# taithenguyen/ppls

Hardware: AMD Instinct MI355X
Metric: accepted subintervals/sec + FP64 F-evals/sec at 1/2/4/8 MI355X, EPSILON=1e-10 (higher is better)
Workload: dtype f64

## Files before the change

### ppls_amd/build.py

```python
import os
import shutil
import subprocess
import sys

HERE = os.path.dirname(os.path.abspath(__file__))
ROOT = os.path.dirname(HERE)
CSRC = os.path.join(HERE, "csrc")
OUT = os.path.join(HERE, "_build")
LIB = os.path.join(OUT, "libaquad.so")
CLI = os.path.join(OUT, "aquad")
HIPCC = shutil.which("hipcc") or "/opt/rocm/bin/hipcc"
ARCH = os.environ.get("PPLS_AMD_ARCH", "gfx950")

HIP_FLAGS = [f"--offload-arch={ARCH}", "-O3", "-std=c++17", "-ffp-contract=off", "-fPIC", "-shared",
             "-mllvm", "-amdgpu-atomic-optimizer-strategy=None",
             "-Wall", "-Wno-unused-function", "-I", os.path.join(ROOT, "include"), "-I", CSRC]

SOURCES = [os.path.join(CSRC, "aquad.hip")]
USER_F = os.path.abspath(os.environ.get("PPLS_AMD_USER_F") or os.path.join(CSRC, "plugins", "aq_user_gauss.h"))
PARAM_F = os.path.abspath(os.environ.get("PPLS_AMD_PARAM_F") or os.path.join(CSRC, "plugins", "aq_param_gauss.h"))
PLUGIN_DEFS = [f'-DAQ_USER_F_HEADER="{USER_F}"', f'-DAQ_PARAM_F_HEADER="{PARAM_F}"']
DEPS = sorted(os.path.join(CSRC, f) for f in os.listdir(CSRC) if f.endswith((".h", ".inc", ".hip"))) + \
    [os.path.join(ROOT, "include", "aquad.h"), USER_F, PARAM_F]
LIBS = ["-pthread", "-L/opt/rocm/lib", "-lrccl", "-Wl,-rpath,/opt/rocm/lib"]


def _stale(target, deps):
    if not os.path.exists(target):
        return True
    t = os.path.getmtime(target)
    return any(os.path.getmtime(d) > t for d in deps)


def build_variant(name, defines, verbose=False):
    os.makedirs(OUT, exist_ok=True)
    out = os.path.join(OUT, f"libaquad_{name}.so")
    cmd = [HIPCC] + HIP_FLAGS + PLUGIN_DEFS + list(defines) + ["-o", out] + SOURCES + LIBS
    if verbose:
        print(" ".join(cmd))
    subprocess.check_call(cmd)
    return out


def build(force=False, verbose=False):
    os.makedirs(OUT, exist_ok=True)
    tab = os.path.join(CSRC, "aq_exp_table.h")
    if not os.path.exists(tab):
        subprocess.check_call([sys.executable, os.path.join(CSRC, "gen_exp_table.py")])
    if not os.path.exists(os.path.join(CSRC, "aq_sincos_table.h")):
        subprocess.check_call([sys.executable, os.path.join(CSRC, "gen_sincos_table.py")])
    if force or _stale(LIB, DEPS):
        cmd = [HIPCC] + HIP_FLAGS + PLUGIN_DEFS + ["-o", LIB] + SOURCES + LIBS
        if verbose:
            print(" ".join(cmd))
        subprocess.check_call(cmd)
    cli_src = os.path.join(CSRC, "aquad_cli.c")
    if os.path.exists(cli_src) and (force or _stale(CLI, [cli_src, LIB])):
        cmd = ["gcc", "-O2", "-std=gnu11", "-Wall", "-I", os.path.join(ROOT, "include"), "-o", CLI, cli_src,
               "-L", OUT, "-laquad", "-Wl,-rpath,$ORIGIN", "-lm"]
        if verbose:
            print(" ".join(cmd))
        subprocess.check_call(cmd)
    return LIB


if __name__ == "__main__":
    if "--variant" in sys.argv:
        i = sys.argv.index("--variant")
        extra = []
        for a in sys.argv[i + 2:]:
            if a.startswith("-D"):
                extra.append(a)
            elif a.startswith("--mllvm="):
                extra += ["-mllvm", a[len("--mllvm="):]]
            elif a.startswith("-f"):
                extra.append(a)
        print("built", build_variant(sys.argv[i + 1], extra))
    else:
        build(force="--force" in sys.argv, verbose=True)
        print("built", LIB)
```

### ppls_amd/csrc/aq_device.h

```cpp
#pragma once
#include <hip/hip_runtime.h>
#include <stdint.h>

#include <type_traits>

#include "aquad.h"
#include "aq_libm.h"

#pragma clang fp contract(off)

namespace aq {

enum : unsigned { ERRB_TIMEOUT = 1, ERRB_OVERFLOW = 2, ERRB_DEPTH = 4 };

__device__ __forceinline__ unsigned cu_slot() {
    const unsigned hw = __builtin_amdgcn_s_getreg((31 << 11) | 4);
    const unsigned xcc = __builtin_amdgcn_s_getreg((3 << 11) | 20);
    const unsigned cu = (hw >> 8) & 15u, sh = (hw >> 12) & 1u, se = (hw >> 13) & 7u;
    return ((xcc & 7u) << 8) | (((se << 1) | sh) << 4) | cu;
}

__device__ __forceinline__ double wave_sum(double v) {
#pragma unroll
    for (int o = 32; o > 0; o >>= 1) v += __shfl_xor(v, o, 64);
    return v;
}
__device__ __forceinline__ unsigned wave_sum_u(unsigned v) {
#pragma unroll
    for (int o = 32; o > 0; o >>= 1) v += __shfl_xor(v, o, 64);
    return v;
}
__device__ __forceinline__ unsigned wave_max_u(unsigned v) {
#pragma unroll
    for (int o = 32; o > 0; o >>= 1) v = max(v, (unsigned)__shfl_xor(v, o, 64));
    return v;
}
__device__ __forceinline__ unsigned wave_or_u(unsigned v) {
#pragma unroll
    for (int o = 32; o > 0; o >>= 1) v |= (unsigned)__shfl_xor((int)v, o, 64);
    return v;
}
__device__ __forceinline__ unsigned lane_id() { return __lane_id(); }
__device__ __forceinline__ unsigned mbcnt(unsigned long long m) {
    return __builtin_amdgcn_mbcnt_hi((unsigned)(m >> 32), __builtin_amdgcn_mbcnt_lo((unsigned)m, 0u));
}

struct Step {
    double mid, fmid, larea, rarea;
    bool refine;
};
template <int FID>
__device__ __forceinline__ Step task_step(double l, double r, double fl, double fr, double eps,
                                          const ExpEntry* __restrict__ tab, const Theta<FID>& th = Theta<FID>{}) {
    Step s;
    const double lrarea = (fl + fr) * (r - l) / 2;
    s.mid = (l + r) / 2;
    s.fmid = integrand<FID>(s.mid, tab, th);
    s.larea = (fl + s.fmid) * (s.mid - l) / 2;
    s.rarea = (s.fmid + fr) * (r - s.mid) / 2;
    s.refine = fabs((s.larea + s.rarea) - lrarea) > eps;
    return s;
}

struct Step2 {
    double fmid, area2;
    bool refine;
};
struct Step2e : Step2 {
    double diff;
};
template <typename S>
constexpr bool step_has_diff = std::is_same<S, Step2e>::value;
template <int FID>
__host__ __device__ constexpr bool doubled_areas() { return FID != F_USER && FID != F_PARAM; }
template <int FID>
__host__ __device__ constexpr double f_scale() { return FID == F_COSH4 ? 16.0 : 1.0; }
template <int FID>
__host__ __device__ constexpr double area_scale() { return doubled_areas<FID>() ? 0.5 / f_scale<FID>() : 1.0; }

template <int FID, int K, typename S = Step2>
__device__ __forceinline__ void task_step_k(const double (&l)[K], const double (&r)[K], const double (&fl)[K],
                                            const double (&fr)[K], double eps2, const ExpEntry* __restrict__ tab,
                                            S (&s)[K], const ExpConsts& kk = ExpConsts{}, int range_hint = -1,
                                            unsigned long long out_mask = 0ull, const Theta<FID>& th = Theta<FID>{}) {
    double mid[K], fmid[K];
#pragma unroll
    for (int k = 0; k < K; ++k) mid[k] = (l[k] + r[k]) / 2;
    double lr2e[K], wl[K], wr[K];
#pragma unroll
    for (int k = 0; k < K; ++k) {
        lr2e[k] = (fl[k] + fr[k]) * (r[k] - l[k]);
        wl[k] = mid[k] - l[k];
        wr[k] = r[k] - mid[k];
        asm volatile("" : "+v"(lr2e[k]), "+v"(wl[k]), "+v"(wr[k]));
    }
    integrand_k<FID, K, (f_scale<FID>() != 1.0)>(mid, fmid, tab, kk, range_hint, out_mask, th);
#pragma unroll
    for (int k = 0; k < K; ++k) {
        if constexpr (doubled_areas<FID>()) {
            const double lr2 = lr2e[k];
            const double l2 = (fl[k] + fmid[k]) * wl[k];
            const double r2 = (fmid[k] + fr[k]) * wr[k];
            s[k].fmid = fmid[k];
            s[k].area2 = l2 + r2;
            s[k].refine = fabs(s[k].area2 - lr2) > eps2;
            if constexpr (step_has_diff<S>) s[k].diff = s[k].area2 - lr2;
        } else {
            const double lrarea = (fl[k] + fr[k]) * (r[k] - l[k]) / 2;
            const double larea = (fl[k] + fmid[k]) * (mid[k] - l[k]) / 2;
            const double rarea = (fmid[k] + fr[k]) * (r[k] - mid[k]) / 2;
            s[k].fmid = fmid[k];
            s[k].area2 = larea + rarea;
            s[k].refine = fabs((larea + rarea) - lrarea) > eps2;
            if constexpr (step_has_diff<S>) s[k].diff = (larea + rarea) - lrarea;
        }
    }
}

template <int FID, unsigned TABMASK = 127u, typename S = Step2>
__device__ __forceinline__ void pair_step_halves(double ha, double hb, double fa, double fm, double fb, double eps2,
                                                 const ExpEntry* __restrict__ tab, S (&s)[2], double& m,
                                                 double& hm, const ExpConsts& kk, int range_hint,
                                                 unsigned long long out_mask, const Theta<FID>& th = Theta<FID>{}) {
    m = ha + hb;
    hm = 0.5 * m;
    const double mid[2] = {ha + hm, hm + hb};
    const double fl[2] = {fa, fm}, fr[2] = {fm, fb};
    double lr2e[2], wl[2], wr[2];
    lr2e[0] = (fa + fm) * __fma_rn(ha, -2.0, m);
    lr2e[1] = (fm + fb) * __fma_rn(hb, 2.0, -m);
    wl[0] = __fma_rn(ha, -2.0, mid[0]);
    wl[1] = mid[1] - m;
    wr[0] = m - mid[0];
    wr[1] = __fma_rn(hb, 2.0, -mid[1]);
#pragma unroll
    for (int k = 0; k < 2; ++k) asm volatile("" : "+v"(lr2e[k]), "+v"(wl[k]), "+v"(wr[k]));
    double fmid[2];
    integrand_k<FID, 2, (f_scale<FID>() != 1.0), TABMASK>(mid, fmid, tab, kk, range_hint, out_mask, th);
#pragma unroll
    for (int k = 0; k < 2; ++k) {
        s[k].fmid = fmid[k];
        if constexpr (doubled_areas<FID>()) {
            const double l2 = (fl[k] + fmid[k]) * wl[k];
            const double r2 = (fmid[k] + fr[k]) * wr[k];
            s[k].area2 = l2 + r2;
            s[k].refine = fabs(s[k].area2 - lr2e[k]) > eps2;
            if constexpr (step_has_diff<S>) s[k].diff = s[k].area2 - lr2e[k];
        } else {
            const double lrarea = lr2e[k] / 2;
            const double larea = (fl[k] + fmid[k]) * wl[k] / 2;
            const double rarea = (fmid[k] + fr[k]) * wr[k] / 2;
            s[k].area2 = larea + rarea;
            s[k].refine = fabs((larea + rarea) - lrarea) > eps2;
            if constexpr (step_has_diff<S>) s[k].diff = (larea + rarea) - lrarea;
        }
    }
}

struct Step2c {
    double fmid, l2, r2, area2;
    bool refine;
};
template <int FID>
__device__ __forceinline__ void pair_step_carry(double ha, double hb, double fa, double fm, double fb, double lr0,
                                                double lr1, double eps2, const ExpEntry* __restrict__ tab,
                                                Step2c (&s)[2], double& m, double& hm, const ExpConsts& kk,
                                                int range_hint, unsigned long long out_mask) {
    static_assert(doubled_areas<FID>(), "carried areas are doubled areas");
    m = ha + hb;
    hm = 0.5 * m;
    const double mid[2] = {ha + hm, hm + hb};
// ... 210 lines not shown
```

### ppls_amd/csrc/aq_libm.h

```cpp
#pragma once
#ifndef AQ_PIN_CONSTS
#define AQ_PIN_CONSTS 1
#endif
#include <hip/hip_runtime.h>
#include <stdint.h>

#include "aquad.h"
#include "aq_exp_table.h"
#include "aq_sincos_table.h"

#pragma clang fp contract(off)

namespace aq {

struct ExpPair {
    uint64_t tail_bits;
    uint64_t sbits;
};
static __constant__ uint64_t kExpTabBits[256] = {AQ_EXP_TAB_INIT};

struct alignas(16) ExpEntry {
    uint64_t tail_bits;
    uint64_t sbits;
};

static constexpr double kInvLn2N = 0x1.71547652b82fep7;
static constexpr double kShift = 0x1.8p52;
static constexpr double kNegLn2hiN = -0x1.62e42fefa0000p-8;
static constexpr double kNegLn2loN = -0x1.cf79abc9e3b3ap-47;
static constexpr double kC2 = 0x1.ffffffffffdbdp-2;
static constexpr double kC3 = 0x1.555555555543cp-3;
static constexpr double kC4 = 0x1.55555cf172b91p-5;
static constexpr double kC5 = 0x1.1111167a4d017p-7;

static constexpr double kQ1 = -3.33333333333331316428e-02;
static constexpr double kQ2 = 1.58730158725481460165e-03;
static constexpr double kQ3 = -7.93650757867487942473e-05;
static constexpr double kQ4 = 4.00821782732936239552e-06;
static constexpr double kQ5 = -2.01099218183624371326e-07;

__device__ __forceinline__ uint32_t hi_word(double x) {
    return (uint32_t)((uint64_t)__double_as_longlong(x) >> 32);
}

__device__ __forceinline__ double exp_glibc(double x, const ExpEntry* __restrict__ tab) {
    double kd = __fma_rn(kInvLn2N, x, kShift);
    const uint64_t ki = (uint64_t)__double_as_longlong(kd);
    kd = kd - kShift;
    const double r = __fma_rn(kd, kNegLn2loN, __fma_rn(kd, kNegLn2hiN, x));
    const ExpEntry e = tab[ki & 127];
    const double tail = __longlong_as_double((long long)e.tail_bits);
    uint64_t sbits = e.sbits + (ki << 45);
    const double r2 = r * r;
    const double tmp = __fma_rn(r2 * r2, __fma_rn(r, kC5, kC4), __fma_rn(r2, __fma_rn(r, kC3, kC2), tail + r));
    if (__builtin_expect(x >= 512.0, 0)) {
        if (x > 0x1.62e42fefa39efp+9) return __longlong_as_double(0x7ff0000000000000LL);
        sbits -= 1009ull << 52;
        const double scale = __longlong_as_double((long long)sbits);
        return 0x1p1009 * __fma_rn(scale, tmp, scale);
    }
    const double scale = __longlong_as_double((long long)sbits);
    return __fma_rn(scale, tmp, scale);
}

__device__ __forceinline__ double exp_glibc_any(double x, const ExpEntry* __restrict__ tab) {
    const uint32_t abstop = (uint32_t)((uint64_t)__double_as_longlong(x) >> 52) & 0x7ffu;
    bool special = false;
    if (__builtin_expect(abstop - 0x3c9u >= 0x408u - 0x3c9u, 0)) {
        if ((int)(abstop - 0x3c9u) < 0) return 1.0 + x;
        if (abstop >= 0x409u) {
            if (__double_as_longlong(x) == (long long)0xfff0000000000000ull) return 0.0;
            if (abstop >= 0x7ffu) return 1.0 + x;
            return x < 0.0 ? 0.0 : __longlong_as_double(0x7ff0000000000000LL);
        }
        special = true;
    }
    double kd = __fma_rn(kInvLn2N, x, kShift);
    const uint64_t ki = (uint64_t)__double_as_longlong(kd);
    kd = kd - kShift;
    const double r = __fma_rn(kd, kNegLn2loN, __fma_rn(kd, kNegLn2hiN, x));
    const ExpEntry e = tab[ki & 127];
    const double tail = __longlong_as_double((long long)e.tail_bits);
    uint64_t sbits = e.sbits + (ki << 45);
// ... 41 lines not shown
#endif
#ifndef AQ_SIN_RECIP_RN
#define AQ_SIN_RECIP_RN 1
#endif
template <int NEWTON = AQ_RCP_NEWTON>
__device__ __forceinline__ double half_recip_n(double t) {
    double y = __builtin_amdgcn_rcp(t);
    if constexpr (NEWTON == 3) {
        const double e = __fma_rn(-t, y, 1.0);
        y = __fma_rn(y, __fma_rn(e, e, e), y);
    } else {
#pragma unroll
        for (int i = 0; i < NEWTON; ++i) {
            const double e = __fma_rn(-t, y, 1.0);
            y = __fma_rn(y, e, y);
        }
    }
    const double q = 0.5 * y;
    const double r = __fma_rn(-t, q, 0.5);
    return __fma_rn(r, y, q);
}
__device__ __forceinline__ double half_recip(double t) { return half_recip_n<>(t); }
__device__ __forceinline__ double recip_rn(double x) {
    double y = __builtin_amdgcn_rcp(x);
#pragma unroll
    for (int i = 0; i < 2; ++i) {
        const double e = __fma_rn(-x, y, 1.0);
        y = __fma_rn(y, e, y);
    }
    const double r = __fma_rn(-x, y, 1.0);
    return __fma_rn(r, y, y);
}

__device__ __forceinline__ double cosh_glibc(double x, const ExpEntry* __restrict__ tab) {
    const uint32_t ix = hi_word(x) & 0x7fffffffu;
    const double ax = fabs(x);
    if (__builtin_expect(ix < 0x40360000u, 1)) {
        if (ix < 0x3fd62e43u) {
            if (ix < 0x3c800000u) return 1.0;
            const double t = expm1_glibc_small(ax);
            const double w = 1.0 + t;
            return 1.0 + (t * t) / (w + w);
        }
        const double t = exp_glibc(ax, tab);
        return __fma_rn(t, 0.5, half_recip(t));
    }
    if (ix >= 0x7ff00000u) return x * x;
    if (ix < 0x40862e42u) return 0.5 * exp_glibc(ax, tab);
    if (ax <= 0x1.633ce8fb9f87dp+9) {
        const double w = exp_glibc(0.5 * ax, tab);
        const double t = 0.5 * w;
        return t * w;
    }
    return __longlong_as_double(0x7ff0000000000000LL);
}

static __constant__ double kSinCosTab[AQ_SINCOS_TAB_N] = {AQ_SINCOS_TAB_INIT};

namespace sinc {
constexpr double s1 = -0x1.5555555555555p-3, s2 = 0.0083333333333323288, s3 = -1.9841269834414642e-04,
                 s4 = 2.755729806860771e-06, s5 = -2.5022014848318398e-08;
constexpr double sn3 = -1.66666666666664880952546298448555E-01, sn5 = 8.33333214285722277379541354343671E-03,
                 cs2 = 4.99999999999999999999950396842453E-01, cs4 = -4.16666666666664434524222570944589E-02,
                 cs6 = 1.38888874007937613028114285595617E-03;
constexpr double big = 0x1.8p45, hp0 = 0x1.921FB54442D18p0, hp1 = 0x1.1A62633145C07p-54, mp1 = 0x1.921FB58p0,
                 mp2 = -0x1.DDE973Cp-27, pp3 = -0x1.CB3B398p-55, pp4 = -0x1.d747f23e32ed7p-83,
                 hpinv = 0x1.45F306DC9C883p-1, toint = 0x1.8p52;
// ... 53 lines not shown
        const double r = (n & 1) ? sin_tab_cos(b, db, st) : sin_tab_sin(b, db, st);
        return (n & 2) ? -r : r;
    }
    return sin(x);
}

__device__ __forceinline__ const double* sin_table(const ExpEntry* tab) { return reinterpret_cast<const double*>(tab); }

enum : int { F_COSH4 = 0, F_SIN_RECIP = 1, F_USER = 2, F_PARAM = 3 };

}

#ifndef AQ_USER_F_HEADER
#define AQ_USER_F_HEADER "plugins/aq_user_gauss.h"
#endif
#include AQ_USER_F_HEADER

#ifndef AQ_PARAM_F_HEADER
#define AQ_PARAM_F_HEADER "plugins/aq_param_gauss.h"
#endif
#include AQ_PARAM_F_HEADER

namespace aq {

static_assert(param::nparams >= 1 && param::nparams <= AQ_MAX_PARAMS, "AQ_F_PARAM: 1 .. AQ_MAX_PARAMS parameters");

template <int FID>
struct Theta {};
template <>
struct Theta<F_PARAM> {
    double v[param::nparams];
};

template <int FID>
__device__ __forceinline__ double integrand(double x, const ExpEntry* __restrict__ tab,
                                            const Theta<FID>& th = Theta<FID>{}) {
    if constexpr (FID == F_COSH4) {
        const double c = cosh_glibc(x, tab);
        return c * c * c * c;
    } else if constexpr (FID == F_USER) {
        return user::F(x, tab);
    } else if constexpr (FID == F_PARAM) {
        return param::F(x, th.v, tab);
    } else {
        return sin_glibc(AQ_SIN_RECIP_RN ? recip_rn(x) : 1.0 / x, sin_table(tab));
    }
}

struct ExpConsts {
    double shift = kShift, c4 = kC4, c2 = kC2;
    double inv = kInvLn2N, hi = kNegLn2hiN, lo = kNegLn2loN, c5 = kC5, c3 = kC3;
};
__device__ __forceinline__ ExpConsts pinned_exp_consts() {
    ExpConsts k;
#if AQ_PIN_CONSTS
    asm volatile("" : "+v"(k.shift), "+v"(k.c4), "+v"(k.c2));
    asm volatile("" : "+v"(k.inv), "+v"(k.hi), "+v"(k.lo), "+v"(k.c5), "+v"(k.c3));
#endif
    return k;
}

__device__ __forceinline__ bool cosh_main_range(double x) {
    const uint32_t ix = hi_word(x) & 0x7fffffffu;
    return ix >= 0x3fd62e43u && ix < 0x40360000u;
}
template <int K, bool CHECK = true, bool TWICE = false, unsigned TABMASK = 127u>
__device__ __forceinline__ bool cosh_main_k(const double (&x)[K], double (&c)[K], const ExpEntry* __restrict__ tab,
                                            const ExpConsts& kk) {
    double ax[K], kd[K], r[K], r2[K], tmp[K], t[K];
    uint64_t ki[K];
    ExpEntry e[K];
    bool out = false;
#pragma unroll
    for (int k = 0; k < K; ++k) {
        ax[k] = fabs(x[k]);
        kd[k] = __fma_rn(kk.inv, ax[k], kk.shift);
        ki[k] = (uint64_t)__double_as_longlong(kd[k]);
        e[k] = tab[ki[k] & TABMASK];
        if (CHECK) out |= !cosh_main_range(x[k]);
    }
#pragma unroll
    for (int k = 0; k < K; ++k) {
        kd[k] = kd[k] - kk.shift;
        r[k] = __fma_rn(kd[k], kk.lo, __fma_rn(kd[k], kk.hi, ax[k]));
        r2[k] = r[k] * r[k];
    }
#pragma unroll
    for (int k = 0; k < K; ++k) {
        const double tail = __longlong_as_double((long long)e[k].tail_bits);
        tmp[k] = __fma_rn(r2[k] * r2[k], __fma_rn(r[k], kk.c5, kk.c4),
                          __fma_rn(r2[k], __fma_rn(r[k], kk.c3, kk.c2), tail + r[k]));
    }
#pragma unroll
    for (int k = 0; k < K; ++k) {
        const uint32_t shi = (uint32_t)(e[k].sbits >> 32) + ((uint32_t)ki[k] << 13);
        const double scale = __hiloint2double((int)shi, (int)(uint32_t)e[k].sbits);
        t[k] = __fma_rn(scale, tmp[k], scale);
    }
    double y[K], q[K];
#pragma unroll
    for (int k = 0; k < K; ++k) y[k] = __builtin_amdgcn_rcp(t[k]);
#pragma unroll
    for (int it = 0; it < 2; ++it) {
#pragma unroll
        for (int k = 0; k < K; ++k) y[k] = __fma_rn(y[k], __fma_rn(-t[k], y[k], 1.0), y[k]);
    }
    if constexpr (TWICE) {
#pragma unroll
        for (int k = 0; k < K; ++k) {
            const double e = __fma_rn(-t[k], y[k], 1.0);
            c[k] = t[k] + __fma_rn(y[k], e, y[k]);
        }
        (void)q;
        return out;
    }
#pragma unroll
    for (int k = 0; k < K; ++k) {
        q[k] = 0.5 * y[k];
        c[k] = __fma_rn(t[k], 0.5, __fma_rn(__fma_rn(-t[k], q[k], 0.5), y[k], q[k]));
    }
    return out;
}

__device__ __forceinline__ bool cosh_main_span(double lo, double hi) {
    return ((int)hi_word(lo) >= 0x3fd62e43) && ((int)hi_word(hi) < 0x40360000);
}
template <int FID, int K, bool SCALED = false, unsigned TABMASK = 127u>
__device__ __forceinline__ void integrand_k(const double (&x)[K], double (&f)[K], const ExpEntry* __restrict__ tab,
                                            const ExpConsts& kk = ExpConsts{}, int range_hint = -1,
                                            unsigned long long out_mask = 0ull, const Theta<FID>& th = Theta<FID>{}) {
    if constexpr (FID == F_COSH4) {
        constexpr double cs = SCALED ? 2.0 : 1.0;
        double c[K];
        bool out;
        if (range_hint == 2) {
            cosh_main_k<K, false, SCALED, TABMASK>(x, c, tab, kk);
            if (__builtin_expect(out_mask != 0ull, 0)) {
#pragma unroll
                for (int k = 0; k < K; ++k)
                    if (!cosh_main_range(x[k])) c[k] = cs * cosh_glibc(x[k], tab);
            }
            out = false;
        } else if (range_hint >= 0) {
            cosh_main_k<K, false, SCALED, TABMASK>(x, c, tab, kk);
            out = range_hint == 0;
        } else {
            out = cosh_main_k<K, true, SCALED, TABMASK>(x, c, tab, kk);
        }
        if (__builtin_expect(__ballot(out) != 0ull, 0)) {
#pragma unroll
            for (int k = 0; k < K; ++k)
                if (!cosh_main_range(x[k])) c[k] = cs * cosh_glibc(x[k], tab);
        }
#pragma unroll
        for (int k = 0; k < K; ++k) f[k] = c[k] * c[k];
#pragma unroll
        for (int k = 0; k < K; ++k) f[k] = f[k] * c[k];
#pragma unroll
        for (int k = 0; k < K; ++k) f[k] = f[k] * c[k];
    } else if constexpr (FID == F_USER) {
#pragma unroll
        for (int k = 0; k < K; ++k) f[k] = user::F(x[k], tab);
    } else if constexpr (FID == F_PARAM) {
#pragma unroll
        for (int k = 0; k < K; ++k) f[k] = param::F(x[k], th.v, tab);
    } else {
#pragma unroll
        for (int k = 0; k < K; ++k) f[k] = sin_glibc(AQ_SIN_RECIP_RN ? recip_rn(x[k]) : 1.0 / x[k], sin_table(tab));
    }
}

template <int FID>
constexpr int ftab_entries() { return FID == F_SIN_RECIP ? (AQ_SINCOS_TAB_N + 1) / 2 : 128; }

__device__ __forceinline__ void stage_exp_table(ExpEntry* lds, const ExpPair* __restrict__ g) {
    for (int i = threadIdx.x; i < 128; i += blockDim.x) {
        lds[i].tail_bits = g[i].tail_bits;
        lds[i].sbits = g[i].sbits;
    }
}
// ... 13 lines not shown
```

### ppls_amd/csrc/aq_stream.h

```cpp
#pragma once
#include "aq_device.h"
#include "aq_shape.h"
#include "aq_xsum.h"

namespace aq {

typedef double f64x2 __attribute__((ext_vector_type(2)));

constexpr int PCAP = 128;
constexpr int DT_STRIDE = 2;
constexpr int LREC = NW * WCAP + PCAP;
constexpr int POOL0 = NW * WCAP;
constexpr int CH = PCAP;
struct DtField {
    unsigned* p;
    __device__ __forceinline__ unsigned& operator[](unsigned j) const { return p[DT_STRIDE * j]; }
    __device__ __forceinline__ DtField operator+(unsigned o) const { return DtField{p + DT_STRIDE * o}; }
};
#ifndef AQ_JOB_RUN_MAX
#define AQ_JOB_RUN_MAX 16
#endif
constexpr int JOB_RUN_MAX = AQ_JOB_RUN_MAX;
#ifndef AQ_GSS_DIV
#define AQ_GSS_DIV 2
// ... 492 lines not shown
        "ds_write2st64_b64 %0, %5, %6 offset0:200 offset1:250"
        :
        : "v"(addr), "v"(r.ab.x), "v"(r.ab.y), "v"(r.ff.x), "v"(r.ff.y), "v"(r.fd.x), "v"(r.fd.y)
        : "memory");
}
__device__ __forceinline__ PairRegs chunk_load(const CellarChunk* ch, unsigned lane) {
    return PairRegs{ch->ab[lane], ch->ff[lane], ch->fd[lane]};
}
__device__ __forceinline__ void chunk_store(CellarChunk* ch, unsigned lane, const PairRegs& r) {
    ch->ab[lane] = r.ab;
    ch->ff[lane] = r.ff;
    ch->fd[lane] = r.fd;
}
__device__ __forceinline__ unsigned ring_addr(unsigned ring8, unsigned i, unsigned vmask) {
    return ((i << 3) & vmask) | ring8;
}
__device__ __forceinline__ unsigned ring_slot(unsigned i) { return i % (unsigned)WCAP; }
__device__ __forceinline__ unsigned ring_wrap(unsigned v) {
    if constexpr ((WCAP & (WCAP - 1)) == 0) return v & (unsigned)(WCAP - 1);
    else return min(v, v - (unsigned)WCAP);
}

#if AQ_STAMPS
__device__ unsigned long long g_aq_stamps[MAXG * NW * ST_STRIDE];
#endif

template <int FID, bool HIST, bool DIAG, bool PCU, int NWT = NW, bool HEAPS = false, bool ERR = false>
__global__ __launch_bounds__(NWT * 64) void k_stream(StreamParams P) {
    static_assert(!ERR || (!HIST && !DIAG), "ERR launches keep no histograms and no diagnostics");
    constexpr int PTT = NWT * 64;
    static_assert(NWT >= 4 && NWT <= NW && NWT % 4 == 0, "whole waves per SIMD, within the LDS rings");
    static_assert(NWT <= 16, "the exit's area sum runs over one DPP row of lanes (PCU_AREA)");
    constexpr bool WIDE = AQ_WIDE_TAB && FID == F_COSH4 && !PCU;
    constexpr int TAB_FRONT = WIDE ? 256 * 16 / 8 : 0;
    __shared__ double s_lds[TAB_FRONT + 6 * LREC];
    double* const s_pr = s_lds + TAB_FRONT;
    __shared__ ExpEntry tab_own[WIDE ? 1 : ftab_entries<FID>()];
    ExpEntry* const tab = WIDE ? reinterpret_cast<ExpEntry*>(s_lds) : tab_own;
    const DtField s_dt{reinterpret_cast<unsigned*>(s_pr + 5 * LREC)};
    double* const s_a = s_pr;
    double* const s_b = s_pr + LREC;
    double* const s_fa = s_pr + 2 * LREC;
    double* const s_fm = s_pr + 3 * LREC;
    double* const s_fb = s_pr + 4 * LREC;
    __shared__ WgState S;
    __shared__ unsigned long long s_pc[PCU ? 3 * PCU_ROW : 1];
    __shared__ double2 s_wdd[PCU ? PCU_ROW * NWT : 1];
    __shared__ double2 s_werr[PCU && ERR ? PCU_ROW * NWT : 1];
    __shared__ unsigned long long s_dg[DIAG ? DIAG_WORDS : 1];

    const unsigned tid = threadIdx.x;
    const unsigned lane = lane_id();
    const unsigned wid = __builtin_amdgcn_readfirstlane(tid >> 6);
    const unsigned bid = __builtin_amdgcn_readfirstlane(blockIdx.x);
    QCtl* __restrict__ qc = P.q;
    const LdsPairs R{s_a, s_b, s_fa, s_fm, s_fb, s_dt};
    const unsigned pr_base = (unsigned)(uintptr_t)s_pr;
    const unsigned long long t_entry = (DIAG || AQ_STAMPS) ? rtc() : 0ull;
    unsigned long long stp[ST_N] = {};
    auto stamp = [&](int k) {
        if constexpr (AQ_STAMPS && !DIAG) { if (!stp[k]) stp[k] = rtc(); }
    };
    stp[ST_ENTRY] = t_entry;
    if constexpr (AQ_STAMPS && !DIAG) {
        asm volatile("" :: "s"(P.eps), "s"(P.shares), "s"(P.nprob), "s"(P.kbounds[0].x));
        stamp(ST_KARG);
    }
    ExpPair tv{};
    if (FID != F_SIN_RECIP && tid < (WIDE ? 256u : 128u)) tv = reinterpret_cast<const ExpPair*>(kExpTabBits)[tid & 127u];
    static_assert(FID != F_SIN_RECIP || AQ_SINCOS_TAB_N <= PTT, "one sin-table entry per thread");
    double sv = 0.0;
    if (FID == F_SIN_RECIP && tid < (unsigned)AQ_SINCOS_TAB_N) sv = kSinCosTab[tid];
    stamp(ST_PRE);
    if (bid == 0)
        for (unsigned i = tid; i < (unsigned)(sizeof(QCtl) / 4); i += PTT) reinterpret_cast<unsigned*>(P.q_next)[i] = 0u;
    if (tid == 0) {
        S.lock = 0; S.pbot = 0; S.ptop = 0; S.idle = 0; S.phase = 0; S.busy_token = 1;
        S.exited = 0; S.tasks = 0;
    }
    if (PCU && tid < 3u * PCU_ROW) s_pc[tid] = 0ull;
    if (PCU)
        for (unsigned i = tid; i < (unsigned)(PCU_ROW * NWT); i += PTT) s_wdd[i] = make_double2(0.0, 0.0);
    if constexpr (PCU && ERR)
        for (unsigned i = tid; i < (unsigned)(PCU_ROW * NWT); i += PTT) s_werr[i] = make_double2(0.0, 0.0);
    if (DIAG) {
        for (unsigned i = tid; i < DIAG_WORDS; i += PTT) s_dg[i] = (i == DG_T_FIRST_LEAD) ? ~0ull : 0ull;
    }
    if (FID == F_SIN_RECIP) {
        if (tid < (unsigned)AQ_SINCOS_TAB_N) reinterpret_cast<double*>(tab)[tid] = sv;
    } else if (tid < (WIDE ? 256u : 128u)) {
        tab[tid].tail_bits = tv.tail_bits;
        tab[tid].sbits = tv.sbits;
    }
    __syncthreads();
    if constexpr (DIAG) { if (tid == 0) s_dg[DG_T_INIT] = rtc(); }
    stamp(ST_INIT);

    const double eps = P.eps;
    const double eps2 = eps / area_scale<FID>();
    const int max_depth = P.max_depth;
    unsigned shares_main = (unsigned)P.shares;
    int D_main = P.D;
    unsigned long long per_hint = 0;
    if (!PCU && (P.adaptive & 1)) {
        unsigned h = uni(__hip_atomic_load(&P.hint->shares_next, __ATOMIC_RELAXED, __HIP_MEMORY_SCOPE_AGENT));
        if (h) {
            if constexpr (HEAPS) {
                const unsigned long long per =
                    (P.adaptive & 4) ? __hip_atomic_load(&P.hint->per_next, __ATOMIC_RELAXED, __HIP_MEMORY_SCOPE_AGENT)
                                     : (h >= 2u ? (unsigned long long)h * TASKS_PER_JOB : 0ull);
                const unsigned fill = (gridDim.x * (unsigned)NWT + (unsigned)P.nprob - 1u) / (unsigned)P.nprob;
                const unsigned long long cap = per / MIN_JOB_TASKS;
                h = uni(max(h, (unsigned)min((unsigned long long)fill, cap)));
                per_hint = per;
            }
            shares_main = h;
            D_main = seed_depth_job((unsigned long long)h * (unsigned long long)P.nshards);
        }
    }
    const unsigned W = gridDim.x * (unsigned)NWT;
    const unsigned w_all = bid * (unsigned)NWT + wid;
    const unsigned grp = bid % (unsigned)NGROUP;
    const unsigned grp_size = (gridDim.x - grp + (unsigned)NGROUP - 1u) / (unsigned)NGROUP;
    const int t0 = (int)min(gridDim.x, (unsigned)NGROUP);
    const unsigned tail_from = (!PCU && shares_main >= 8u) ? (unsigned)P.tail_from : (unsigned)P.nprob;
// ... 874 lines not shown
        };
        window();
        constexpr bool prio_by_load = PCU && FID == F_SIN_RECIP;
        const bool b_heavy = prio_by_load && b_S >= HEAVY_S;
        const unsigned b_max = give_rounds - b_poll % give_rounds;
        unsigned b_rem = b_max;
        __builtin_amdgcn_s_waitcnt(0xC07F);
        bool b_go;
        for (;;) {
        for (;;) {
            unsigned long long c0 = 0, c1 = 0;
            if constexpr (DIAG) c0 = clk();
            if constexpr (prio_by_load) {
                if (b_heavy) asm volatile("s_setprio 3");
                else asm volatile("s_setprio 1");
            }
            const unsigned long long need = ~b_am;
            const unsigned k = min((unsigned)__popcll(need), b_top - b_bot);
            const unsigned jr = mbcnt(need);
            const unsigned long long fmsk = __ballot(jr < k) & need;
            b_top -= k;
            const unsigned paddr = ring_addr(ring8, ring_slot(b_top) + jr, ring_vmask);
            lds_pop6_masked(fmsk, paddr, paddr + 3u * 50u * 512u, ca, cb, cfa, cfm, cfb, cdw);
            const unsigned long long am = b_am | fmsk;
            const unsigned na = (unsigned)__popcll(am);
            const double pa = ca, pb = cb, pfa = cfa, pfm = cfm, pfb = cfb;
            const unsigned long long dtw = (unsigned long long)__double_as_longlong(cdw);
            const unsigned dt = (unsigned)dtw;
            using StepT = typename std::conditional<ERR, Step2e, Step2>::type;
            StepT st[2];
            unsigned long long nospan = 0ull;
            if constexpr (FID == F_COSH4) nospan = __ballot((int)dt >= 0);
            double pm, hm;
            pair_step_halves<FID, WIDE ? 255u : 127u, StepT>(pa, pb, pfa, pfm, pfb, eps2, tab, st, pm, hm, kk,
                                                              FID == F_COSH4 ? 2 : -1, nospan & am, th);
            if constexpr (prio_by_load) { if (!b_heavy) asm volatile("s_setprio 0"); }
            const unsigned long long r0m = __ballot(st[0].refine), r1m = __ballot(st[1].refine);
            unsigned long long okm = am;
            if constexpr (!burst_cap) {
                const unsigned long long dm = __ballot((dt & 255u) < (unsigned)(max_depth - 1));
                okm = am & dm;
                const unsigned long long atcap = am & ~dm;
                if (__builtin_expect(atcap != 0ull, 0)) b_dv |= atcap & (r0m | r1m);
            }
            const unsigned long long l0m = am & ~r0m, l1m = am & ~r1m;
            b_n += na;
            const unsigned long long mask0 = okm & r0m, mask1 = okm & r1m;
            const unsigned cdt = dt + 1u;
            const unsigned long long cdtw = ((dtw >> 32) << 32) | (unsigned long long)cdt;
            masked_acc3(acc.r, st[0].area2, l0m, st[1].area2, l1m, acc.maxdt, burst_cap ? cdt : dt,
                        burst_cap ? (mask0 | mask1) : am);
            if constexpr (ERR) masked_err4(eacc.sg, eacc.ab, st[0].diff, l0m, st[1].diff, l1m);
            if constexpr (DIAG) {
                const int rtag = (int)dt_tag(dt);
                b_mixed |= (__ballot(rtag != tag) & am) != 0ull;
            }
            if (HIST) {
                const unsigned d = dt & 255u;
                if (__builtin_amdgcn_inverse_ballot_w64(am)) {
                    atomicAdd(&P.ctls[P.first_slot + tag].hist[d], 2ull);
                    const unsigned nl = ((l0m >> lane) & 1u) + ((l1m >> lane) & 1u);
                    if (nl) atomicAdd(&P.ctls[P.first_slot + tag].hist[AQ_MAX_LEVELS + d], (unsigned long long)nl);
                }
            }
            if constexpr (DIAG) c1 = clk();
            lds_push6_masked(mask1, ring_addr(ring8, ring_slot(b_top) + mbcnt(mask1), ring_vmask), hm, pb, pfm,
                             st[1].fmid, pfb, __longlong_as_double((long long)cdtw));
// ... 218 lines not shown
```

### ppls_amd/csrc/aquad.hip

```cpp
#include <hip/hip_runtime.h>

#include <algorithm>
#include <atomic>
#include <chrono>
#include <condition_variable>
#include <cmath>
#include <cstdio>
#include <cstdlib>
#include <cstring>
#include <functional>
#include <memory>
#include <mutex>
#include <string>
#include <thread>
#include <type_traits>
#include <vector>

#include "aquad.h"
#include "aq_exp_table.h"
#include "aq_libm.h"
#include "aq_device.h"
#include "aq_stream.h"
#include "aq_launch_plan.h"
#include "aq_host_pool.h"

#include <rccl/rccl.h>

#pragma clang fp contract(off)

namespace aq {

struct DevResults {
    double area;
    unsigned long long tasks;
    unsigned long long leaves;
    unsigned long long spilled;
    unsigned int levels;
    unsigned int error;
    unsigned long long tasks_per_level[AQ_MAX_LEVELS];
    unsigned long long leaves_per_level[AQ_MAX_LEVELS];
    unsigned long long cu_tasks[AQ_CU_SLOTS];
};


template <int FID, bool COSH_ONLY>
__global__ __launch_bounds__(256) void k_eval(const double* __restrict__ x, double* __restrict__ out, size_t n,
                                              const ExpPair* __restrict__ gtab) {
    constexpr int TF = COSH_ONLY ? F_COSH4 : FID;
    __shared__ ExpEntry tab[ftab_entries<TF>()];
    stage_f_table<TF>(tab, gtab);
    __syncthreads();
    const size_t gid = (size_t)blockIdx.x * blockDim.x + threadIdx.x, stride = (size_t)gridDim.x * blockDim.x;
    if constexpr (FID == F_COSH4 && !COSH_ONLY) {
        const ExpConsts kk = pinned_exp_consts();
        for (size_t i = 2 * gid; i < n; i += 2 * stride) {
            const double xx[2] = {x[i], x[i + 1 < n ? i + 1 : i]};
            double ff[2];
            integrand_k<F_COSH4, 2, true>(xx, ff, tab, kk);
            out[i] = ff[0] / f_scale<F_COSH4>();
            if (i + 1 < n) out[i + 1] = ff[1] / f_scale<F_COSH4>();
        }
    } else {
        for (size_t i = gid; i < n; i += stride) out[i] = COSH_ONLY ? cosh_glibc(x[i], tab) : integrand<FID>(x[i], tab);
    }
}

__global__ __launch_bounds__(256) void k_eval_params(const double* __restrict__ x, const double* __restrict__ theta,
                                                     double* __restrict__ out, size_t n,
                                                     const ExpPair* __restrict__ gtab) {
    __shared__ ExpEntry tab[ftab_entries<F_PARAM>()];
    stage_f_table<F_PARAM>(tab, gtab);
    __syncthreads();
    const size_t gid = (size_t)blockIdx.x * blockDim.x + threadIdx.x, stride = (size_t)gridDim.x * blockDim.x;
    for (size_t i = gid; i < n; i += stride) {
        Theta<F_PARAM> th;
#pragma unroll
        for (int j = 0; j < param::nparams; ++j) th.v[j] = theta[i * param::nparams + j];
        out[i] = integrand<F_PARAM>(x[i], tab, th);
    }
}

constexpr int EST_KEYS = 256;
constexpr double EST_PER_OCTAVE = 8.0;
constexpr double EST_TASKS = 2.84;
template <int FID>
// ... 671 lines not shown
```

Baseline: 300.6 billion.

## Seed cosh reciprocal from a 2^(-i/128) table instead of hardware rcp

Adds a table of 2^(-i/128) values that is stored next to the exp table entries in LDS, widening each entry to 32 bytes. In the hot cosh path, the reciprocal of exp(x) is now seeded from this table plus a short polynomial in r, followed by two Newton steps. This replaces the v_rcp_f64 hardware estimate and its refinement sequence. The trade-off is a larger LDS table footprint and extra loads in exchange for a cheaper, more accurate seed.

```diff
diff --git a/ppls_amd/build.py b/ppls_amd/build.py
--- a/ppls_amd/build.py
+++ b/ppls_amd/build.py
@@ -47,6 +47,8 @@
     tab = os.path.join(CSRC, "aq_exp_table.h")
     if not os.path.exists(tab):
         subprocess.check_call([sys.executable, os.path.join(CSRC, "gen_exp_table.py")])
+    if not os.path.exists(os.path.join(CSRC, "aq_inv_table.h")):
+        subprocess.check_call([sys.executable, os.path.join(CSRC, "gen_inv_table.py")])
     if not os.path.exists(os.path.join(CSRC, "aq_sincos_table.h")):
         subprocess.check_call([sys.executable, os.path.join(CSRC, "gen_sincos_table.py")])
     if force or _stale(LIB, DEPS):
diff --git a/ppls_amd/csrc/aq_device.h b/ppls_amd/csrc/aq_device.h
--- a/ppls_amd/csrc/aq_device.h
+++ b/ppls_amd/csrc/aq_device.h
@@ -49,9 +49,9 @@
     double mid, fmid, larea, rarea;
     bool refine;
 };
-template <int FID>
+template <int FID, class E>
 __device__ __forceinline__ Step task_step(double l, double r, double fl, double fr, double eps,
-                                          const ExpEntry* __restrict__ tab, const Theta<FID>& th = Theta<FID>{}) {
+                                          const E* __restrict__ tab, const Theta<FID>& th = Theta<FID>{}) {
     Step s;
     const double lrarea = (fl + fr) * (r - l) / 2;
     s.mid = (l + r) / 2;
@@ -117,9 +117,9 @@
     }
 }
 
-template <int FID, unsigned TABMASK = 127u, typename S = Step2>
+template <int FID, unsigned TABMASK = 127u, typename S = Step2, bool SEED = false, class E>
 __device__ __forceinline__ void pair_step_halves(double ha, double hb, double fa, double fm, double fb, double eps2,
-                                                 const ExpEntry* __restrict__ tab, S (&s)[2], double& m,
+                                                 const E* __restrict__ tab, S (&s)[2], double& m,
                                                  double& hm, const ExpConsts& kk, int range_hint,
                                                  unsigned long long out_mask, const Theta<FID>& th = Theta<FID>{}) {
     m = ha + hb;
@@ -136,7 +136,7 @@
 #pragma unroll
     for (int k = 0; k < 2; ++k) asm volatile("" : "+v"(lr2e[k]), "+v"(wl[k]), "+v"(wr[k]));
     double fmid[2];
-    integrand_k<FID, 2, (f_scale<FID>() != 1.0), TABMASK>(mid, fmid, tab, kk, range_hint, out_mask, th);
+    integrand_k<FID, 2, (f_scale<FID>() != 1.0), TABMASK, SEED>(mid, fmid, tab, kk, range_hint, out_mask, th);
 #pragma unroll
     for (int k = 0; k < 2; ++k) {
         s[k].fmid = fmid[k];
diff --git a/ppls_amd/csrc/aq_inv_table.h b/ppls_amd/csrc/aq_inv_table.h
--- /dev/null
+++ b/ppls_amd/csrc/aq_inv_table.h
@@ -0,0 +1,69 @@
+#pragma once
+#include <stdint.h>
+#define AQ_INV_TAB_INIT \
+    0x3ff0000000000000ULL, 0x3feff3c22b8f71f1ULL, \
+    0x3fefe7c1819e90d8ULL, 0x3fefdbfdad9cbe14ULL, \
+    0x3fefd0765b6e4540ULL, 0x3fefc52b376bba97ULL, \
+    0x3fefba1bee615a27ULL, 0x3fefaf482d8e67f1ULL, \
+    0x3fefa4afa2a490daULL, 0x3fef9a51fbc74c83ULL, \
+    0x3fef902ee78b3ff6ULL, 0x3fef864614f5a129ULL, \
+    0x3fef7c97337b9b5fULL, 0x3fef7321f301b460ULL, \
+    0x3fef69e603db3285ULL, 0x3fef60e316c98398ULL, \
+    0x3fef5818dcfba487ULL, 0x3fef4f87080d89f2ULL, \
+    0x3fef472d4a07897cULL, 0x3fef3f0b555dc3faULL, \
+    0x3fef3720dcef9069ULL, 0x3fef2f6d9406e7b5ULL, \
+    0x3fef27f12e57d14bULL, 0x3fef20ab5fffd07aULL, \
+    0x3fef199bdd85529cULL, 0x3fef12c25bd71e09ULL, \
+    0x3fef0c1e904bc1d2ULL, 0x3fef05b030a1064aULL, \
+    0x3feeff76f2fb5e47ULL, 0x3feef9728de5593aULL, \
+    0x3feef3a2b84f15fbULL, 0x3feeee07298db666ULL, \
+    0x3feee89f995ad3adULL, 0x3feee36bbfd3f37aULL, \
+    0x3feede6b5579fdbfULL, 0x3feed99e1330b358ULL, \
+    0x3feed503b23e255dULL, 0x3feed09bec4a2d33ULL, \
+    0x3feecc667b5de565ULL, 0x3feec86319e32323ULL, \
+    0x3feec49182a3f090ULL, 0x3feec0f170ca07baULL, \
+    0x3feebd829fde4e50ULL, 0x3feeba44cbc8520fULL, \
+    0x3feeb737b0cdc5e5ULL, 0x3feeb45b0b91ffc6ULL, \
+    0x3feeb1ae99157736ULL, 0x3feeaf3216b5448cULL, \
+    0x3feeace5422aa0dbULL, 0x3feeaac7d98a6699ULL, \
+    0x3feea8d99b4492edULL, 0x3feea71a4623c7adULL, \
+    0x3feea589994cce13ULL, 0x3feea427543e1a12ULL, \
+    0x3feea2f336cf4e62ULL, 0x3feea1ed0130c132ULL, \
+    0x3feea11473eb0187ULL, 0x3feea0694fde5d3fULL, \
+    0x3fee9feb564267c9ULL, 0x3fee9f9a48a58174ULL, \
+    0x3fee9f75e8ec5f74ULL, 0x3fee9f7df9519484ULL, \
+    0x3fee9fb23c651a2fULL, 0x3feea012750bdabfULL, \
+    0x3feea09e667f3bcdULL, 0x3feea155d44ca973ULL, \
+    0x3feea23882552225ULL, 0x3feea34634ccc320ULL, \
+    0x3feea47eb03a5585ULL, 0x3feea5e1b976dc09ULL, \
+    0x3feea76f15ad2148ULL, 0x3feea9268a5946b7ULL, \
+    0x3feeab07dd485429ULL, 0x3feead12d497c7fdULL, \
+    0x3feeaf4736b527daULL, 0x3feeb1a4ca5d920fULL, \
+    0x3feeb42b569d4f82ULL, 0x3feeb6daa2cf6642ULL, \
+    0x3feeb9b2769d2ca7ULL, 0x3feebcb299fddd0dULL, \
+    0x3feebfdad5362a27ULL, 0x3feec32af0d7d3deULL, \
+    0x3feec6a2b5c13cd0ULL, 0x3feeca41ed1d0057ULL, \
+    0x3feece086061892dULL, 0x3feed1f5d950a897ULL, \
+    0x3feed60a21f72e2aULL, 0x3feeda4504ac801cULL, \
+    0x3feedea64c123422ULL, 0x3feee32dc313a8e5ULL, \
+    0x3feee7db34e59ff7ULL, 0x3feeecae6d05d866ULL, \
+    0x3feef1a7373aa9cbULL, 0x3feef6c55f929ff1ULL, \
+    0x3feefc08b26416ffULL, 0x3fef0170fc4cd831ULL, \
+    0x3fef06fe0a31b715ULL, 0x3fef0cafa93e2f56ULL, \
+    0x3fef1285a6e4030bULL, 0x3fef187fd0dad990ULL, \
+    0x3fef1e9df51fdee1ULL, 0x3fef24dfe1f56381ULL, \
+    0x3fef2b4565e27cddULL, 0x3fef31ce4fb2a63fULL, \
+    0x3fef387a6e756238ULL, 0x3fef3f49917ddc96ULL, \
+    0x3fef463b88628cd6ULL, 0x3fef4d5022fcd91dULL, \
+    0x3fef54873168b9aaULL, 0x3fef5be084045cd4ULL, \
+    0x3fef635beb6fcb75ULL, 0x3fef6af9388c8deaULL, \
+    0x3fef72b83c7d517bULL, 0x3fef7a98c8a58e51ULL, \
+    0x3fef829aaea92de0ULL, 0x3fef8abdc06c31ccULL, \
+    0x3fef9301d0125b51ULL, 0x3fef9b66affed31bULL, \
+    0x3fefa3ec32d3d1a2ULL, 0x3fefac922b7247f7ULL, \
+    0x3fefb5586cf9890fULL, 0x3fefbe3ecac6f383ULL, \
+    0x3fefc74518759bc8ULL, 0x3fefd06b29ddf6deULL, \
+    0x3fefd9b0d3158574ULL, 0x3fefe315e86e7f85ULL, \
+    0x3fefec9a3e778061ULL, 0x3feff63da9fb3335ULL, \
+
+static const uint64_t aq_inv_tab_host[128] = {AQ_INV_TAB_INIT};
diff --git a/ppls_amd/csrc/aq_libm.h b/ppls_amd/csrc/aq_libm.h
--- a/ppls_amd/csrc/aq_libm.h
+++ b/ppls_amd/csrc/aq_libm.h
@@ -2,11 +2,18 @@
 #ifndef AQ_PIN_CONSTS
 #define AQ_PIN_CONSTS 1
 #endif
+#ifndef AQ_RCP_SEED
+#define AQ_RCP_SEED 1
+#endif
 #include <hip/hip_runtime.h>
 #include <stdint.h>
 
+#include <type_traits>
+
 #include "aquad.h"
 #include "aq_exp_table.h"
+#include "aq_inv_table.h"
+#include "aq_rcp_seed.h"
 #include "aq_sincos_table.h"
 
 #pragma clang fp contract(off)
@@ -19,10 +26,20 @@
 };
 static __constant__ uint64_t kExpTabBits[256] = {AQ_EXP_TAB_INIT};
 
+static __constant__ uint64_t kInvTabBits[128] = {AQ_INV_TAB_INIT};
+
 struct alignas(16) ExpEntry {
     uint64_t tail_bits;
     uint64_t sbits;
 };
+struct alignas(32) ExpEntryInv {
+    uint64_t tail_bits;
+    uint64_t sbits;
+    uint64_t inv_bits;
+    uint64_t pad;
+};
+template <class E>
+constexpr bool has_inv = std::is_same<E, ExpEntryInv>::value;
 
 static constexpr double kInvLn2N = 0x1.71547652b82fep7;
 static constexpr double kShift = 0x1.8p52;
@@ -43,12 +60,13 @@
     return (uint32_t)((uint64_t)__double_as_longlong(x) >> 32);
 }
 
-__device__ __forceinline__ double exp_glibc(double x, const ExpEntry* __restrict__ tab) {
+template <class E>
+__device__ __forceinline__ double exp_glibc(double x, const E* __restrict__ tab) {
     double kd = __fma_rn(kInvLn2N, x, kShift);
     const uint64_t ki = (uint64_t)__double_as_longlong(kd);
     kd = kd - kShift;
     const double r = __fma_rn(kd, kNegLn2loN, __fma_rn(kd, kNegLn2hiN, x));
-    const ExpEntry e = tab[ki & 127];
+    const E e = tab[ki & 127];
     const double tail = __longlong_as_double((long long)e.tail_bits);
     uint64_t sbits = e.sbits + (ki << 45);
     const double r2 = r * r;
@@ -156,7 +174,8 @@
     return __fma_rn(r, y, y);
 }
 
-__device__ __forceinline__ double cosh_glibc(double x, const ExpEntry* __restrict__ tab) {
+template <class E>
+__device__ __forceinline__ double cosh_glibc(double x, const E* __restrict__ tab) {
     const uint32_t ix = hi_word(x) & 0x7fffffffu;
     const double ax = fabs(x);
     if (__builtin_expect(ix < 0x40360000u, 1)) {
@@ -276,8 +295,8 @@
     double v[param::nparams];
 };
 
-template <int FID>
-__device__ __forceinline__ double integrand(double x, const ExpEntry* __restrict__ tab,
+template <int FID, class E>
+__device__ __forceinline__ double integrand(double x, const E* __restrict__ tab,
                                             const Theta<FID>& th = Theta<FID>{}) {
     if constexpr (FID == F_COSH4) {
         const double c = cosh_glibc(x, tab);
@@ -308,12 +327,13 @@
     const uint32_t ix = hi_word(x) & 0x7fffffffu;
     return ix >= 0x3fd62e43u && ix < 0x40360000u;
 }
-template <int K, bool CHECK = true, bool TWICE = false, unsigned TABMASK = 127u>
-__device__ __forceinline__ bool cosh_main_k(const double (&x)[K], double (&c)[K], const ExpEntry* __restrict__ tab,
+template <int K, bool CHECK = true, bool TWICE = false, unsigned TABMASK = 127u, bool SEED = false, class E>
+__device__ __forceinline__ bool cosh_main_k(const double (&x)[K], double (&c)[K], const E* __restrict__ tab,
                                             const ExpConsts& kk) {
+    static_assert(!SEED || (TWICE && has_inv<E>), "the seeded reciprocal: 2 cosh from a table with 2^(-i/128)");
     double ax[K], kd[K], r[K], r2[K], tmp[K], t[K];
     uint64_t ki[K];
-    ExpEntry e[K];
+    E e[K];
     bool out = false;
 #pragma unroll
     for (int k = 0; k < K; ++k) {
@@ -342,6 +362,22 @@
         t[k] = __fma_rn(scale, tmp[k], scale);
     }
     double y[K], q[K];
+    if constexpr (SEED) {
+        int m13 = -8192;
+        asm("" : "+s"(m13));
+#pragma unroll
+        for (int k = 0; k < K; ++k) {
+            const uint32_t ihi = (uint32_t)((int)(uint32_t)(e[k].inv_bits >> 32) + __mul24((int)(uint32_t)ki[k], m13));
+            const double inv = __hiloint2double((int)ihi, (int)(uint32_t)e[k].inv_bits);
+            y[k] = rcp_seed(r[k], r2[k], inv, kNegSixth);
+        }
+#pragma unroll
+        for (int k = 0; k < K; ++k) y[k] = rcp_newton(t[k], y[k]);
+#pragma unroll
+        for (int k = 0; k < K; ++k) c[k] = t[k] + rcp_newton(t[k], y[k]);
+        (void)q;
+        return out;
+    }
 #pragma unroll
     for (int k = 0; k < K; ++k) y[k] = __builtin_amdgcn_rcp(t[k]);
 #pragma unroll
@@ -369,8 +405,8 @@
 __device__ __forceinline__ bool cosh_main_span(double lo, double hi) {
     return ((int)hi_word(lo) >= 0x3fd62e43) && ((int)hi_word(hi) < 0x40360000);
 }
-template <int FID, int K, bool SCALED = false, unsigned TABMASK = 127u>
-__device__ __forceinline__ void integrand_k(const double (&x)[K], double (&f)[K], const ExpEntry* __restrict__ tab,
+template <int FID, int K, bool SCALED = false, unsigned TABMASK = 127u, bool SEED = false, class E>
+__device__ __forceinline__ void integrand_k(const double (&x)[K], double (&f)[K], const E* __restrict__ tab,
                                             const ExpConsts& kk = ExpConsts{}, int range_hint = -1,
                                             unsigned long long out_mask = 0ull, const Theta<FID>& th = Theta<FID>{}) {
     if constexpr (FID == F_COSH4) {
@@ -378,7 +414,7 @@
         double c[K];
         bool out;
         if (range_hint == 2) {
-            cosh_main_k<K, false, SCALED, TABMASK>(x, c, tab, kk);
+            cosh_main_k<K, false, SCALED, TABMASK, SEED>(x, c, tab, kk);
             if (__builtin_expect(out_mask != 0ull, 0)) {
 #pragma unroll
                 for (int k = 0; k < K; ++k)
@@ -386,10 +422,10 @@
             }
             out = false;
         } else if (range_hint >= 0) {
-            cosh_main_k<K, false, SCALED, TABMASK>(x, c, tab, kk);
+            cosh_main_k<K, false, SCALED, TABMASK, SEED>(x, c, tab, kk);
             out = range_hint == 0;
         } else {
-            out = cosh_main_k<K, true, SCALED, TABMASK>(x, c, tab, kk);
+            out = cosh_main_k<K, true, SCALED, TABMASK, SEED>(x, c, tab, kk);
         }
         if (__builtin_expect(__ballot(out) != 0ull, 0)) {
 #pragma unroll
diff --git a/ppls_amd/csrc/aq_rcp_seed.h b/ppls_amd/csrc/aq_rcp_seed.h
--- /dev/null
+++ b/ppls_amd/csrc/aq_rcp_seed.h
@@ -0,0 +1,24 @@
+#pragma once
+
+#if defined(__HIPCC__) || defined(__CUDACC__)
+#define AQ_HD __host__ __device__ __forceinline__
+#else
+#define AQ_HD inline
+#endif
+
+namespace aq {
+
+static constexpr double kNegSixth = -0x1.5555555555555p-3;
+
+AQ_HD double rcp_seed(double r, double r2, double inv, double neg_sixth) {
+    const double q1 = __builtin_fma(r, neg_sixth, 0.5);
+    const double p = __builtin_fma(r2, q1, -r);
+    return __builtin_fma(inv, p, inv);
+}
+
+AQ_HD double rcp_newton(double t, double y) { return __builtin_fma(y, __builtin_fma(-t, y, 1.0), y); }
+
+AQ_HD double rcp_seed_recip(double t, double y0) { return rcp_newton(t, rcp_newton(t, y0)); }
+AQ_HD double rcp_seed_sum(double t, double y0) { return t + rcp_seed_recip(t, y0); }
+
+}
diff --git a/ppls_amd/csrc/aq_stream.h b/ppls_amd/csrc/aq_stream.h
--- a/ppls_amd/csrc/aq_stream.h
+++ b/ppls_amd/csrc/aq_stream.h
@@ -548,11 +548,14 @@
     static_assert(NWT >= 4 && NWT <= NW && NWT % 4 == 0, "whole waves per SIMD, within the LDS rings");
     static_assert(NWT <= 16, "the exit's area sum runs over one DPP row of lanes (PCU_AREA)");
     constexpr bool WIDE = AQ_WIDE_TAB && FID == F_COSH4 && !PCU;
-    constexpr int TAB_FRONT = WIDE ? 256 * 16 / 8 : 0;
+    constexpr bool SEED = AQ_RCP_SEED && WIDE && !DIAG;
+    using TabT = std::conditional_t<SEED, ExpEntryInv, ExpEntry>;
+    constexpr int TAB_FRONT = WIDE ? 256 * (int)sizeof(TabT) / 8 : 0;
+    static_assert(TAB_FRONT * 8 % 2048 == 0, "the pair block starts on a multiple of a ring's 2 KiB per field");
     __shared__ double s_lds[TAB_FRONT + 6 * LREC];
     double* const s_pr = s_lds + TAB_FRONT;
     __shared__ ExpEntry tab_own[WIDE ? 1 : ftab_entries<FID>()];
-    ExpEntry* const tab = WIDE ? reinterpret_cast<ExpEntry*>(s_lds) : tab_own;
+    TabT* const tab = WIDE ? reinterpret_cast<TabT*>(s_lds) : reinterpret_cast<TabT*>(tab_own);
     const DtField s_dt{reinterpret_cast<unsigned*>(s_pr + 5 * LREC)};
     double* const s_a = s_pr;
     double* const s_b = s_pr + LREC;
@@ -585,6 +588,8 @@
     ExpPair tv{};
     if (FID != F_SIN_RECIP && tid < (WIDE ? 256u : 128u)) tv = reinterpret_cast<const ExpPair*>(kExpTabBits)[tid & 127u];
     static_assert(FID != F_SIN_RECIP || AQ_SINCOS_TAB_N <= PTT, "one sin-table entry per thread");
+    uint64_t tiv = 0;
+    if (SEED && tid < 256u) tiv = kInvTabBits[tid & 127u];
     double sv = 0.0;
     if (FID == F_SIN_RECIP && tid < (unsigned)AQ_SINCOS_TAB_N) sv = kSinCosTab[tid];
     stamp(ST_PRE);
@@ -607,6 +612,7 @@
     } else if (tid < (WIDE ? 256u : 128u)) {
         tab[tid].tail_bits = tv.tail_bits;
         tab[tid].sbits = tv.sbits;
+        if constexpr (SEED) tab[tid].inv_bits = tiv;
     }
     __syncthreads();
     if constexpr (DIAG) { if (tid == 0) s_dg[DG_T_INIT] = rtc(); }
@@ -1547,7 +1553,7 @@
             unsigned long long nospan = 0ull;
             if constexpr (FID == F_COSH4) nospan = __ballot((int)dt >= 0);
             double pm, hm;
-            pair_step_halves<FID, WIDE ? 255u : 127u, StepT>(pa, pb, pfa, pfm, pfb, eps2, tab, st, pm, hm, kk,
+            pair_step_halves<FID, WIDE ? 255u : 127u, StepT, SEED>(pa, pb, pfa, pfm, pfb, eps2, tab, st, pm, hm, kk,
                                                               FID == F_COSH4 ? 2 : -1, nospan & am, th);
             if constexpr (prio_by_load) { if (!b_heavy) asm volatile("s_setprio 0"); }
             const unsigned long long r0m = __ballot(st[0].refine), r1m = __ballot(st[1].refine);
diff --git a/ppls_amd/csrc/aquad.hip b/ppls_amd/csrc/aquad.hip
--- a/ppls_amd/csrc/aquad.hip
+++ b/ppls_amd/csrc/aquad.hip
@@ -47,10 +47,28 @@
 __global__ __launch_bounds__(256) void k_eval(const double* __restrict__ x, double* __restrict__ out, size_t n,
                                               const ExpPair* __restrict__ gtab) {
     constexpr int TF = COSH_ONLY ? F_COSH4 : FID;
+    const size_t gid = (size_t)blockIdx.x * blockDim.x + threadIdx.x, stride = (size_t)gridDim.x * blockDim.x;
+    if constexpr (FID == F_COSH4 && !COSH_ONLY && AQ_RCP_SEED && AQ_WIDE_TAB) {
+        __shared__ ExpEntryInv tabw[256];
+        for (unsigned i = threadIdx.x; i < 256u; i += blockDim.x) {
+            tabw[i].tail_bits = gtab[i & 127u].tail_bits;
+            tabw[i].sbits = gtab[i & 127u].sbits;
+            tabw[i].inv_bits = kInvTabBits[i & 127u];
+        }
+        __syncthreads();
+        const ExpConsts kk = pinned_exp_consts();
+        for (size_t i = 2 * gid; i < n; i += 2 * stride) {
+            const double xx[2] = {x[i], x[i + 1 < n ? i + 1 : i]};
+            double ff[2];
+            integrand_k<F_COSH4, 2, true, 255u, true>(xx, ff, tabw, kk);
+            out[i] = ff[0] / f_scale<F_COSH4>();
+            if (i + 1 < n) out[i + 1] = ff[1] / f_scale<F_COSH4>();
+        }
+        return;
+    }
     __shared__ ExpEntry tab[ftab_entries<TF>()];
     stage_f_table<TF>(tab, gtab);
     __syncthreads();
-    const size_t gid = (size_t)blockIdx.x * blockDim.x + threadIdx.x, stride = (size_t)gridDim.x * blockDim.x;
     if constexpr (FID == F_COSH4 && !COSH_ONLY) {
         const ExpConsts kk = pinned_exp_consts();
         for (size_t i = 2 * gid; i < n; i += 2 * stride) {
diff --git a/ppls_amd/csrc/gen_inv_table.py b/ppls_amd/csrc/gen_inv_table.py
--- /dev/null
+++ b/ppls_amd/csrc/gen_inv_table.py
@@ -0,0 +1,38 @@
+import decimal
+import os
+import struct
+
+N = 128
+
+
+def _bits(x: float) -> int:
+    return struct.unpack("<Q", struct.pack("<d", x))[0]
+
+
+def table():
+    ctx = decimal.Context(prec=100)
+    two = decimal.Decimal(2)
+    out = []
+    for i in range(N):
+        exact = ctx.power(two, ctx.divide(decimal.Decimal(-i), decimal.Decimal(N)))
+        out.append((_bits(float(exact)) + ((i << 52) // N)) & 0xFFFFFFFFFFFFFFFF)
+    return out
+
+
+def main():
+    tab = table()
+    path = os.path.join(os.path.dirname(os.path.abspath(__file__)), "aq_inv_table.h")
+    with open(path, "w") as f:
+        f.write("// GENERATED by ppls_amd/csrc/gen_inv_table.py -- do not edit.\n")
+        f.write("// bits(RN(2^(-i/128))) + (i << 45), i = 0..127 (the seeded reciprocal, aq_rcp_seed.h).\n")
+        f.write("#pragma once\n#include <stdint.h>\n")
+        f.write("#define AQ_INV_TAB_INIT \\\n")
+        for i in range(0, N, 2):
+            f.write("    0x%016xULL, 0x%016xULL, \\\n" % (tab[i], tab[i + 1]))
+        f.write("\n")
+        f.write("static const uint64_t aq_inv_tab_host[%d] = {AQ_INV_TAB_INIT};\n" % N)
+    print("wrote", path)
+
+
+if __name__ == "__main__":
+    main()
```

Result: no change. 302.1 billion, median of 6 (+0.5%).
